# mx-mark/VideoTransformer-pytorch

Measured on NVIDIA H100. Metric: clips/sec (BxTx3x224x224) TimeSformer-B fwd+bwd, higher is better.
Workload: dtype bf16

## Files before the change

### videotransformer_pytorch_b200/csrc/vt_gemm.cu

```cuda
#include <stdlib.h>
#include <string.h>

#include "vt_common.cuh"
#include "vt_sm90.cuh"

namespace vt {

constexpr int BM = 128;
constexpr int BK = 64;
constexpr int GEMM_THREADS = 384;
constexpr int CHUNK_BYTES = 64 * BK * 2;

struct GemmDev {
  int M, N, K;
  int kblocks, splits;
  int num_m, num_n, tiles;
  int epi;
  const float* bias;
  const float* bias2;
  void* out;
  void* out2;
  const void* aux;
  long long ldo, ldo2, ldaux;
  const int* out_row;
  const int* aux_row;
  const float* row_scale;
  long long split_stride;
  int map_period, map_skip, map_tcount;
  long long map_stride_t, map_stride_p, map_stride_b, map_base;
  float* special_out;
  long long special_ld;
  const float* a_scale;
  const float* b_scale;
};

constexpr int EPI_BOX_BYTES = 64 * 64 * 2;

template <int BN, int SE>
struct GemmCfg {
  static constexpr int A_BYTES = BM * BK * 2;
  static constexpr int B_BYTES = BN * BK * 2;
  static constexpr int STAGE_BYTES = A_BYTES + B_BYTES;
  static constexpr int EPI_TILE_BYTES = BM * BN * 2;
  static constexpr int EPI_BYTES = SE * EPI_TILE_BYTES;
  static constexpr int SMEM_LIMIT = 232448, SMEM_EXTRA = 1024  + 256 ;
  static constexpr int STAGES_FIT = (SMEM_LIMIT - SMEM_EXTRA - EPI_BYTES) / STAGE_BYTES;
  static constexpr int STAGES = STAGES_FIT < 6 ? STAGES_FIT : 6;
  static constexpr int SMEM_BYTES = STAGES * STAGE_BYTES + EPI_BYTES + SMEM_EXTRA;
  static_assert(STAGES >= 2 && SMEM_BYTES <= SMEM_LIMIT, "shared memory budget");
};

template <int BN, int TA, int TB>
__device__ __forceinline__ void wgmma_tile(float (&acc)[BN / 2], uint64_t da, uint64_t db, uint32_t scale_d) {
  if constexpr (BN == 256) wgmma_m64n256k16<TA, TB>(acc, da, db, scale_d);
  else if constexpr (BN == 192) wgmma_m64n192k16<TA, TB>(acc, da, db, scale_d);
  else wgmma_m64n128k16<TA, TB>(acc, da, db, scale_d);
}

struct EpiRow {
  char* out;
  const char* aux;
  char* out2;
  float s;
};

__device__ __forceinline__ EpiRow epi_row(const GemmDev& p, int row, int split) {
  EpiRow r{nullptr, nullptr, nullptr, 1.0f};
  if (row >= p.M) return r;
  if (p.row_scale) r.s = p.row_scale[row];
  if (p.epi == VT_EPI_F32) {
    float* out = static_cast<float*>(p.out);
    const float* aux = static_cast<const float*>(p.aux);
    if (p.map_period > 0) {
      const int outer = row / p.map_period, inner = row - outer * p.map_period;
      if (inner < p.map_skip) {
        if (p.special_out) r.out = reinterpret_cast<char*>(p.special_out + (long long)outer * p.special_ld);
        return r;
      }
      const long long off = p.map_base + (long long)(outer % p.map_tcount) * p.map_stride_t +
                            (long long)(inner - p.map_skip) * p.map_stride_p + (long long)(outer / p.map_tcount) * p.map_stride_b;
      r.out = reinterpret_cast<char*>(out + off);
      r.aux = reinterpret_cast<const char*>(aux + off);
      return r;
    }
    const int orow = p.out_row ? p.out_row[row] : row;
    if (orow >= 0) r.out = reinterpret_cast<char*>(out + (long long)split * p.split_stride + (long long)orow * p.ldo);
    if (aux) {
      const int arow = p.aux_row ? p.aux_row[row] : row;
      if (arow >= 0) r.aux = reinterpret_cast<const char*>(aux + (long long)arow * p.ldaux);
    }
    return r;
  }
  const int orow = p.out_row ? p.out_row[row] : row;
  if (orow < 0) return r;
  r.out = reinterpret_cast<char*>(static_cast<__nv_bfloat16*>(p.out) + (long long)orow * p.ldo);
  if (p.epi == VT_EPI_GELU) r.out2 = reinterpret_cast<char*>(static_cast<__nv_bfloat16*>(p.out2) + (long long)orow * p.ldo2);
  if (p.epi == VT_EPI_DGELU) r.aux = reinterpret_cast<const char*>(static_cast<const __nv_bfloat16*>(p.aux) + (long long)row * p.ldaux);
// ... 44 lines not shown
__device__ __forceinline__ void epi_stage(const GemmDev& p, const float (&acc)[BN / 2], uint8_t* stage, uint8_t* stage2,
                                          int row0, int n0, int warp, int lane) {
  const int r = warp * 16 + (lane >> 2);
  float s[2] = {1.0f, 1.0f};
  if ((EPI == VT_EPI_BF16 || EPI == VT_EPI_GELU_H) && p.row_scale) {
#pragma unroll
    for (int h = 0; h < 2; ++h)
      if (row0 + r + 8 * h < p.M) s[h] = p.row_scale[row0 + r + 8 * h];
  }
  const uint32_t a1 = smem_u32(stage) + r * 128 + 4 * (lane & 3) + ((lane >> 2) << 4);
  const uint32_t a2 = smem_u32(stage2) + r * 128 + 4 * (lane & 3) + ((lane >> 2) << 4);
#pragma unroll
  for (int j = 0; j < BN / 8; ++j) {
    const int n = n0 + 8 * j + 2 * (lane & 3);
    if (n >= p.N) break;
#pragma unroll
    for (int h = 0; h < 2; ++h) {
      const uint32_t off = (j >> 3) * EPI_BOX_BYTES + h * 8 * 128;
      const uint32_t o = (a1 ^ ((j & 7) << 4)) + off, o2 = (a2 ^ ((j & 7) << 4)) + off;
      float v0 = acc[4 * j + 2 * h], v1 = acc[4 * j + 2 * h + 1];
      add_bias(p, n, v0, v1);
      if (EPI == VT_EPI_BF16) {
        st_shared_u32(o, pack_bf16x2(s[h] * v0, s[h] * v1));
      } else if (EPI == VT_EPI_GELU_H) {
        st_shared_u32(o, gelu_pair(pack_bf16x2(s[h] * v0, s[h] * v1)));
      } else if (EPI == VT_EPI_GELU) {
        const uint32_t z = pack_bf16x2(v0, v1);
        st_shared_u32(o, z);
        st_shared_u32(o2, gelu_pair(z));
      } else {
        st_shared_u32(o, dgelu_pair(ld_shared_u32(o2), v0, v1));
      }
    }
  }
}

struct Tile {
  int m0, n0, split, kb0, kb1;
};

template <int BN>
__device__ __forceinline__ Tile tile_at(const GemmDev& p, int t) {
  Tile c;
  const int nt = t % p.num_n, rest = t / p.num_n;
  const int mt = rest % p.num_m;
  c.split = rest / p.num_m;
  c.m0 = mt * BM;
  c.n0 = nt * BN;
  c.kb0 = (int)(((long long)p.kblocks * c.split) / p.splits);
  c.kb1 = (int)(((long long)p.kblocks * (c.split + 1)) / p.splits);
  return c;
}

template <int BN, int TA, int TB, int SE, int F8>
__device__ __forceinline__ void gemm_wgmma_body(const CUtensorMap& tmA, const CUtensorMap& tmB, const CUtensorMap& tmC,
                                                const CUtensorMap& tmD, const GemmDev& p) {
  using Cfg = GemmCfg<BN, SE>;
  static_assert(!F8 || (BN == 128 && !TA && !TB && SE < 2), "e4m3 forms: BN = 128, K-major operands, one output");
  constexpr int STAGES = Cfg::STAGES;
  constexpr int KB_ELEMS = F8 ? 128 : BK;
  constexpr int HALF_BYTES = Cfg::EPI_TILE_BYTES / 2;
  extern __shared__ uint8_t smem_raw[];
  uint8_t* smem = reinterpret_cast<uint8_t*>((reinterpret_cast<uintptr_t>(smem_raw) + 1023) & ~uintptr_t(1023));
  uint8_t* epi_smem = smem + STAGES * Cfg::STAGE_BYTES;
  uint64_t* full_bar = reinterpret_cast<uint64_t*>(epi_smem + Cfg::EPI_BYTES);
  uint64_t* empty_bar = full_bar + STAGES;
  uint64_t* zfull_bar = empty_bar + STAGES;
  uint64_t* zempty_bar = zfull_bar + 1;
  const bool load_z = SE == 2 && p.epi == VT_EPI_DGELU;

  const int wg = threadIdx.x >> 7;
  if (threadIdx.x == 0) {
    tma_prefetch_desc(&tmA);
    tma_prefetch_desc(&tmB);
    if (SE > 0) tma_prefetch_desc(&tmC);
    if (SE == 2) tma_prefetch_desc(&tmD);
    for (int i = 0; i < STAGES; ++i) {
      mbar_init(&full_bar[i], 1);
      mbar_init(&empty_bar[i], 8);
    }
    mbar_init(zfull_bar, 1);
    mbar_init(zempty_bar, 2);
    fence_barrier_init();
  }
  __syncthreads();

  if (wg == 0) {
    setmaxnreg_dec<40>();
    if (threadIdx.x == 0) {
      uint32_t it = 0;
      uint32_t tj = 0;
      for (int t = blockIdx.x; t < p.tiles; t += gridDim.x, ++tj) {
        const Tile c = tile_at<BN>(p, t);
        for (int kb = c.kb0; kb < c.kb1; ++kb, ++it) {
          const int stage = (int)(it % STAGES);
          mbar_wait(&empty_bar[stage], ((it / STAGES) & 1) ^ 1);
          uint8_t* sA = smem + stage * Cfg::STAGE_BYTES;
          uint8_t* sB = sA + Cfg::A_BYTES;
          mbar_arrive_expect_tx(&full_bar[stage], Cfg::STAGE_BYTES);
          if (!TA) {
            tma_load_2d(sA, &tmA, &full_bar[stage], kb * KB_ELEMS, c.m0);
          } else {
#pragma unroll
            for (int ch = 0; ch < BM / 64; ++ch) tma_load_2d(sA + ch * CHUNK_BYTES, &tmA, &full_bar[stage], c.m0 + ch * 64, kb * BK);
          }
          if (!TB) {
            tma_load_2d(sB, &tmB, &full_bar[stage], kb * KB_ELEMS, c.n0);
          } else {
#pragma unroll
            for (int ch = 0; ch < BN / 64; ++ch) tma_load_2d(sB + ch * CHUNK_BYTES, &tmB, &full_bar[stage], c.n0 + ch * 64, kb * BK);
          }
        }
        if (load_z) {
          mbar_wait(zempty_bar, (tj & 1) ^ 1);
          mbar_arrive_expect_tx(zfull_bar, Cfg::EPI_TILE_BYTES);
          uint8_t* zt = epi_smem + Cfg::EPI_TILE_BYTES;
#pragma unroll
          for (int h = 0; h < 2; ++h)
#pragma unroll
            for (int b = 0; b < BN / 64; ++b)
              tma_load_2d(zt + h * HALF_BYTES + b * EPI_BOX_BYTES, &tmD, zfull_bar, c.n0 + 64 * b, c.m0 + 64 * h);
        }
      }
    }
    return;
  }

  setmaxnreg_inc<232>();
  const int cw = wg - 1;
  const int warp = (threadIdx.x >> 5) & 3, lane = threadIdx.x & 31;
  const bool leader = (threadIdx.x & 127) == 0;
  uint8_t* stage = epi_smem + cw * HALF_BYTES;
  uint8_t* stage2 = stage + Cfg::EPI_TILE_BYTES;
  uint32_t it = 0, tj = 0;
  float part[F8 ? BN / 2 : 1];
#pragma unroll
  for (int i = 0; i < (F8 ? BN / 2 : 1); ++i) part[i] = 0.f;
  for (int t = blockIdx.x; t < p.tiles; t += gridDim.x, ++tj) {
    const Tile c = tile_at<BN>(p, t);
    float acc[BN / 2];
#pragma unroll
    for (int i = 0; i < BN / 2; ++i) acc[i] = 0.f;
    if constexpr (F8) {
      for (int kb = c.kb0; kb < c.kb1; ++kb, ++it) {
        const int stage = (int)(it % STAGES);
        mbar_wait(&full_bar[stage], (it / STAGES) & 1);
        const uint32_t a_addr = smem_u32(smem + stage * Cfg::STAGE_BYTES) + cw * 64 * 128;
        const uint32_t b_addr = smem_u32(smem + stage * Cfg::STAGE_BYTES + Cfg::A_BYTES);
        wgmma_fence();
#pragma unroll
        for (int k = 0; k < 4; ++k)
          wgmma_m64n128k32_e4m3(part, sdesc_kmajor(a_addr + k * 32), sdesc_kmajor(b_addr + k * 32), k > 0 ? 1u : 0u);
        wgmma_commit();
        wgmma_wait<0>();
        if (lane == 0) mbar_arrive(&empty_bar[stage]);
#pragma unroll
        for (int i = 0; i < BN / 2; ++i) acc[i] += part[i];
      }
      const int rr = c.m0 + cw * 64 + warp * 16 + (lane >> 2);
      const float sa0 = rr < p.M ? p.a_scale[rr] : 0.f, sa1 = rr + 8 < p.M ? p.a_scale[rr + 8] : 0.f;
#pragma unroll
      for (int j = 0; j < BN / 8; ++j) {
        const int n = c.n0 + 8 * j + 2 * (lane & 3);
        if (n >= p.N) break;
        const float2 sb = __ldg(reinterpret_cast<const float2*>(p.b_scale + n));
        acc[4 * j] *= sa0 * sb.x;
        acc[4 * j + 1] *= sa0 * sb.y;
        acc[4 * j + 2] *= sa1 * sb.x;
        acc[4 * j + 3] *= sa1 * sb.y;
      }
    } else {
    int prev = -1;
    for (int kb = c.kb0; kb < c.kb1; ++kb, ++it) {
      const int stage = (int)(it % STAGES);
      mbar_wait(&full_bar[stage], (it / STAGES) & 1);
      const uint32_t a_addr = smem_u32(smem + stage * Cfg::STAGE_BYTES) + cw * (TA ? CHUNK_BYTES : 64 * 128);
      const uint32_t b_addr = smem_u32(smem + stage * Cfg::STAGE_BYTES + Cfg::A_BYTES);
      wgmma_fence();
#pragma unroll
      for (int k = 0; k < BK / 16; ++k) {
        const uint64_t da = TA ? sdesc_mnmajor(a_addr + k * 2048, CHUNK_BYTES) : sdesc_kmajor(a_addr + k * 32);
        const uint64_t db = TB ? sdesc_mnmajor(b_addr + k * 2048, CHUNK_BYTES) : sdesc_kmajor(b_addr + k * 32);
        wgmma_tile<BN, TA, TB>(acc, da, db, (kb > c.kb0 || k > 0) ? 1u : 0u);
      }
      wgmma_commit();
      wgmma_wait<1>();
      if (prev >= 0 && lane == 0) mbar_arrive(&empty_bar[prev]);
      prev = stage;
    }
    wgmma_wait<0>();
    if (lane == 0) mbar_arrive(&empty_bar[prev]);
    }

    if constexpr (SE > 0) {
      const int row0 = c.m0 + cw * 64;
      if (load_z) mbar_wait(zfull_bar, tj & 1);
      if (leader) tma_store_wait_read_all();
      named_bar_sync(1 + cw, 128);
      if (SE == 1 && p.epi == VT_EPI_GELU_H) epi_stage<BN, VT_EPI_GELU_H>(p, acc, stage, stage2, row0, c.n0, warp, lane);
      else if (SE == 1) epi_stage<BN, VT_EPI_BF16>(p, acc, stage, stage2, row0, c.n0, warp, lane);
      else if (p.epi == VT_EPI_GELU) epi_stage<BN, VT_EPI_GELU>(p, acc, stage, stage2, row0, c.n0, warp, lane);
      else epi_stage<BN, VT_EPI_DGELU>(p, acc, stage, stage2, row0, c.n0, warp, lane);
      fence_proxy_async_smem();
      named_bar_sync(1 + cw, 128);
      if (leader) {
        if (load_z) mbar_arrive(zempty_bar);
        if (row0 < p.M) {
#pragma unroll
          for (int b = 0; b < BN / 64; ++b) {
            if (c.n0 + 64 * b >= p.N) break;
            tma_store_2d(&tmC, stage + b * EPI_BOX_BYTES, c.n0 + 64 * b, row0);
            if (SE == 2 && p.epi == VT_EPI_GELU) tma_store_2d(&tmD, stage2 + b * EPI_BOX_BYTES, c.n0 + 64 * b, row0);
          }
        }
        tma_store_commit();
      }
    } else {
      const int r0 = c.m0 + cw * 64 + warp * 16 + (lane >> 2);
      const EpiRow e0 = epi_row(p, r0, c.split), e1 = epi_row(p, r0 + 8, c.split);
#pragma unroll
      for (int j = 0; j < BN / 8; ++j) {
        const int n = c.n0 + 8 * j + 2 * (lane & 3);
        if (n >= p.N) break;
        epi_pair(p, e0, n, acc[4 * j], acc[4 * j + 1]);
        epi_pair(p, e1, n, acc[4 * j + 2], acc[4 * j + 3]);
      }
    }
  }
  if (SE > 0 && leader) tma_store_wait_read_all();
}

template <int BN, int TA, int TB, int SE>
__global__ void __launch_bounds__(GEMM_THREADS, 1)
gemm_wgmma_kernel(const __grid_constant__ CUtensorMap tmA, const __grid_constant__ CUtensorMap tmB,
                  const __grid_constant__ CUtensorMap tmC, const __grid_constant__ CUtensorMap tmD, const GemmDev p) {
  gemm_wgmma_body<BN, TA, TB, SE, 0>(tmA, tmB, tmC, tmD, p);
}

template <int SE>
__global__ void __launch_bounds__(GEMM_THREADS, 1)
gemm_e4m3_kernel(const __grid_constant__ CUtensorMap tmA, const __grid_constant__ CUtensorMap tmB,
                 const __grid_constant__ CUtensorMap tmC, const __grid_constant__ CUtensorMap tmD, const GemmDev p) {
  gemm_wgmma_body<128, 0, 0, SE, 1>(tmA, tmB, tmC, tmD, p);
}

typedef CUresult (*EncodeTiledFn)(CUtensorMap*, CUtensorMapDataType, cuuint32_t, void*, const cuuint64_t*,
                                  const cuuint64_t*, const cuuint32_t*, const cuuint32_t*, CUtensorMapInterleave,
                                  CUtensorMapSwizzle, CUtensorMapL2promotion, CUtensorMapFloatOOBfill);

static EncodeTiledFn get_encode_fn() {
  static EncodeTiledFn fn = nullptr;
  if (!fn) {
    void* ptr = nullptr;
    cudaDriverEntryPointQueryResult qres;
    cudaError_t e = cudaGetDriverEntryPoint("cuTensorMapEncodeTiled", &ptr, cudaEnableDefault, &qres);
    if (e != cudaSuccess || qres != cudaDriverEntryPointSuccess || !ptr) return nullptr;
    fn = reinterpret_cast<EncodeTiledFn>(ptr);
  }
  return fn;
}

static int make_tmap_2d(CUtensorMap* map, int esize, const void* base, long long rows, long long cols, long long ld,
                        int box_rows) {
  EncodeTiledFn fn = get_encode_fn();
  VT_REQUIRE(fn != nullptr, "cuTensorMapEncodeTiled entry point unavailable");
  VT_REQUIRE((reinterpret_cast<uintptr_t>(base) & 15) == 0, "TMA base pointer must be 16-byte aligned");
  VT_REQUIRE((ld * esize) % 16 == 0, "TMA leading dimension must be a multiple of %d elements (got %lld)", 16 / esize, ld);
  cuuint64_t gdim[2] = {(cuuint64_t)cols, (cuuint64_t)rows};
  cuuint64_t gstr[1] = {(cuuint64_t)(ld * esize)};
  cuuint32_t box[2] = {(cuuint32_t)(128 / esize), (cuuint32_t)box_rows};
  cuuint32_t estr[2] = {1u, 1u};
  CUresult r = fn(map, esize == 2 ? CU_TENSOR_MAP_DATA_TYPE_BFLOAT16 : CU_TENSOR_MAP_DATA_TYPE_UINT8, 2, const_cast<void*>(base),
                  gdim, gstr, box, estr,
                  CU_TENSOR_MAP_INTERLEAVE_NONE, CU_TENSOR_MAP_SWIZZLE_128B, CU_TENSOR_MAP_L2_PROMOTION_L2_256B,
                  CU_TENSOR_MAP_FLOAT_OOB_FILL_NONE);
  VT_REQUIRE(r == CUDA_SUCCESS, "cuTensorMapEncodeTiled failed (%d) rows=%lld cols=%lld ld=%lld box_rows=%d", (int)r,
             rows, cols, ld, box_rows);
  return 0;
}

int make_tmap_bf16_2d(CUtensorMap* map, const void* base, long long rows, long long cols, long long ld, int box_rows) {
  return make_tmap_2d(map, 2, base, rows, cols, ld, box_rows);
}

__global__ void reduce_rows_kernel(const float* __restrict__ in, float* __restrict__ out, long long stride, int S,
                                   long long n4, int accumulate, float scale) {
  for (long long i = blockIdx.x * (long long)blockDim.x + threadIdx.x; i < n4; i += (long long)gridDim.x * blockDim.x) {
    float4 acc = make_float4(0.f, 0.f, 0.f, 0.f);
    for (int s = 0; s < S; ++s) {
// ... 15 lines not shown
reduce_rows_tall_kernel(const float* __restrict__ in, float* __restrict__ out, long long stride, int S, long long n4,
                        int accumulate, float scale) {
  const int cq = threadIdx.x % RT_QUADS, rl = threadIdx.x / RT_QUADS;
  const long long i = blockIdx.x * (long long)RT_QUADS + cq;
  float4 acc = make_float4(0.f, 0.f, 0.f, 0.f);
  if (i < n4) {
    for (int s = rl; s < S; s += RT_LANES) {
      const float4 v = *reinterpret_cast<const float4*>(in + (long long)s * stride + i * 4);
      acc.x += v.x; acc.y += v.y; acc.z += v.z; acc.w += v.w;
    }
  }
  __shared__ float4 sh[RT_LANES][RT_QUADS];
  sh[rl][cq] = acc;
  __syncthreads();
  if (rl < 16) {
    float4 a = sh[rl][cq];
#pragma unroll
    for (int r = rl + 16; r < RT_LANES; r += 16) { a.x += sh[r][cq].x; a.y += sh[r][cq].y; a.z += sh[r][cq].z; a.w += sh[r][cq].w; }
    sh[rl][cq] = a;
  }
  __syncthreads();
  if (rl == 0 && i < n4) {
    float4 a = sh[0][cq];
#pragma unroll
    for (int r = 1; r < 16; ++r) { a.x += sh[r][cq].x; a.y += sh[r][cq].y; a.z += sh[r][cq].z; a.w += sh[r][cq].w; }
    a.x *= scale; a.y *= scale; a.z *= scale; a.w *= scale;
    float4* o = reinterpret_cast<float4*>(out + i * 4);
    if (accumulate) { const float4 p = *o; a.x += p.x; a.y += p.y; a.z += p.z; a.w += p.w; }
    *o = a;
  }
}

int launch_reduce_rows(const float* in, float* out, long long stride, int S, long long n, int accumulate, float scale,
                       cudaStream_t st) {
  VT_REQUIRE(n % 4 == 0 && stride % 4 == 0, "vt_reduce_rows: n and stride must be multiples of 4");
  const long long n4 = n / 4;
  if (S >= 32 && n4 <= 16 * 4096) {
    reduce_rows_tall_kernel<<<(int)((n4 + RT_QUADS - 1) / RT_QUADS), RT_QUADS * RT_LANES, 0, st>>>(in, out, stride, S, n4, accumulate, scale);
    return check_launch("reduce_rows_tall_kernel");
  }
  int blocks = (int)((n4 + 255) / 256);
  const int cap = sm_count() * 8;
  if (blocks > cap) blocks = cap;
  if (blocks < 1) blocks = 1;
  reduce_rows_kernel<<<blocks, 256, 0, st>>>(in, out, stride, S, n4, accumulate, scale);
  return check_launch("reduce_rows_kernel");
}

template <int BN, int TA, int TB, int SE, int F8 = 0>
static int launch_gemm_t(const CUtensorMap (&tm)[4], const GemmDev& d, cudaStream_t st) {
  using Cfg = GemmCfg<BN, SE>;
  void (*kernel)(const CUtensorMap, const CUtensorMap, const CUtensorMap, const CUtensorMap, const GemmDev);
  if constexpr (F8) kernel = gemm_e4m3_kernel<SE>;
  else kernel = gemm_wgmma_kernel<BN, TA, TB, SE>;
  static bool attr_set = false;
  if (!attr_set) {
    cudaError_t e = cudaFuncSetAttribute(kernel, cudaFuncAttributeMaxDynamicSharedMemorySize, Cfg::SMEM_BYTES);
    VT_REQUIRE(e == cudaSuccess, "cudaFuncSetAttribute(smem=%d) failed: %s", Cfg::SMEM_BYTES, cudaGetErrorString(e));
    attr_set = true;
  }
  const int grid = d.tiles < persistent_sm_count() ? d.tiles : persistent_sm_count();
  kernel<<<grid, GEMM_THREADS, Cfg::SMEM_BYTES, st>>>(tm[0], tm[1], tm[2], tm[3], d);
  return check_launch(F8 ? "gemm_e4m3_kernel" : "gemm_wgmma_kernel");
}

template <int BN, int SE>
static int launch_layout(const vt_gemm_params* q, const CUtensorMap (&tm)[4], const GemmDev& d, cudaStream_t st) {
  if (!q->a_mn_major && !q->b_mn_major) return launch_gemm_t<BN, 0, 0, SE>(tm, d, st);
  if (!q->a_mn_major) return launch_gemm_t<BN, 0, 1, SE>(tm, d, st);
  if (!q->b_mn_major) return launch_gemm_t<BN, 1, 0, SE>(tm, d, st);
  return launch_gemm_t<BN, 1, 1, SE>(tm, d, st);
}

#ifndef VT_DEFAULT_STAGED_EPI
#define VT_DEFAULT_STAGED_EPI true
#endif
static int staged_kind(const vt_gemm_params* q) {
  if (q->epilogue == VT_EPI_F32 || q->out_row) return 0;
  if (!feature_on("VT_GEMM_STAGED_EPI", VT_DEFAULT_STAGED_EPI)) return 0;
  if (q->epilogue == VT_EPI_BF16 || q->epilogue == VT_EPI_GELU_H) return 1;
  if (q->epilogue == VT_EPI_GELU && ((reinterpret_cast<uintptr_t>(q->out2) & 15) || (q->ldo2 * 2) % 16)) return 0;
  return 2;
}

template <int BN, int F8 = 0>
static int launch_gemm(const vt_gemm_params* q, GemmDev& d, cudaStream_t st) {
  CUtensorMap tm[4];
  memset(tm, 0, sizeof(tm));
  CUtensorMap &tmA = tm[0], &tmB = tm[1];
  int rc;
  if (F8) {
    rc = make_tmap_2d(&tmA, 1, q->a, q->M, q->K, q->lda, BM);
    if (!rc) rc = make_tmap_2d(&tmB, 1, q->b, q->N, q->K, q->ldb, BN);
  } else if (!q->a_mn_major) rc = make_tmap_bf16_2d(&tmA, q->a, q->M, q->K, q->lda, BM);
  else rc = make_tmap_bf16_2d(&tmA, q->a, q->K, q->M, q->lda, BK);
  if (rc) return rc;
  if (!F8) {
    if (!q->b_mn_major) rc = make_tmap_bf16_2d(&tmB, q->b, q->N, q->K, q->ldb, BN);
    else rc = make_tmap_bf16_2d(&tmB, q->b, q->K, q->N, q->ldb, BK);
    if (rc) return rc;
  }
  d.num_m = (q->M + BM - 1) / BM;
  d.num_n = (q->N + BN - 1) / BN;
  const long long tiles = (long long)d.num_m * d.num_n * d.splits;
  VT_REQUIRE(tiles < (1LL << 31), "vt_gemm: M=%d N=%d gives too many tiles", q->M, q->N);
  d.tiles = (int)tiles;
  const long long tile_out = (long long)q->M * q->N;
  void* final_out = d.out;
  d.split_stride = 0;
  if (d.splits > 1) {
    d.out = q->workspace;
    d.ldo = q->N;
    d.split_stride = tile_out;
  }
  const int se = d.splits > 1 ? 0 : staged_kind(q);
  if (se > 0) {
    rc = make_tmap_bf16_2d(&tm[2], q->out, q->M, q->N, q->ldo, 64);
    if (!rc && q->epilogue == VT_EPI_GELU) rc = make_tmap_bf16_2d(&tm[3], q->out2, q->M, q->N, q->ldo2, 64);
    if (!rc && q->epilogue == VT_EPI_DGELU) rc = make_tmap_bf16_2d(&tm[3], q->aux, q->M, q->N, q->ldaux, 64);
    if (rc) return rc;
  }
  if constexpr (F8) {
    rc = se == 1 ? launch_gemm_t<BN, 0, 0, 1, 1>(tm, d, st) : launch_gemm_t<BN, 0, 0, 0, 1>(tm, d, st);
  } else {
    if (se == 1) rc = launch_layout<BN, 1>(q, tm, d, st);
    else if (se == 2) rc = launch_layout<BN, 2>(q, tm, d, st);
    else rc = launch_layout<BN, 0>(q, tm, d, st);
  }
  if (rc) return rc;
  if (d.splits > 1) {
    VT_REQUIRE(q->ldo == q->N, "vt_gemm: split-K requires ldo == N");
    return launch_reduce_rows(static_cast<const float*>(q->workspace), static_cast<float*>(final_out), tile_out, d.splits, tile_out,
                              0, 1.0f, st);
  }
  return 0;
}

int launch_gemm_rows(const vt_gemm_params* q, int m0, void* stream);

}

#ifndef VT_DEFAULT_ROWS_SPLIT
#define VT_DEFAULT_ROWS_SPLIT false
#endif
static int rows_split_point(const vt_gemm_params* q) {
  const int r = q->M % vt::BM;
  if (r == 0 || r > 16 || q->M < 8 * vt::BM) return 0;
  if (q->N > 1024 || q->K < 2048) return 0;
  if (!vt::feature_on("VT_ROWS_SPLIT", VT_DEFAULT_ROWS_SPLIT)) return 0;
  if (q->a_mn_major || (q->epilogue != VT_EPI_BF16 && q->epilogue != VT_EPI_F32)) return 0;
  if (q->out_row || q->aux_row || q->map_period > 0 || q->debug || q->force_splits || q->force_bn || q->force_cluster || q->force_tail) return 0;
  if (q->epilogue == VT_EPI_F32 && q->workspace && !q->aux && !q->bias && !q->row_scale) return 0;
  if (q->K % 8 != 0 || q->lda % 8 != 0 || q->ldb % 8 != 0) return 0;
  if ((reinterpret_cast<uintptr_t>(q->a) & 15) || (reinterpret_cast<uintptr_t>(q->b) & 15)) return 0;
  return q->M - r;
}

static int gemm_dispatch(const vt_gemm_params* q, const float* a_scale, const float* b_scale, void* stream);

extern "C" int vt_gemm(const vt_gemm_params* q, void* stream) {
  using namespace vt;
  VT_REQUIRE(q != nullptr, "vt_gemm: null params");
  const int m0 = (q->a && q->b && q->out && q->M > 0 && q->N > 0 && q->K > 0) ? rows_split_point(q) : 0;
  if (m0 > 0) {
    vt_gemm_params head = *q;
    head.M = m0;
    const int rc = gemm_dispatch(&head, nullptr, nullptr, stream);
    if (rc) return rc;
    return launch_gemm_rows(q, m0, stream);
  }
  return gemm_dispatch(q, nullptr, nullptr, stream);
}

extern "C" int vt_gemm_e4m3(const vt_gemm_e4m3_params* p, void* stream) {
  using namespace vt;
  VT_REQUIRE(p != nullptr, "vt_gemm_e4m3: null params");
  const vt_gemm_params* q = &p->g;
  VT_REQUIRE(p->a_scale && p->b_scale && (reinterpret_cast<uintptr_t>(p->b_scale) & 15) == 0,
             "vt_gemm_e4m3: a_scale and b_scale are required (b_scale 16-byte aligned)");
  VT_REQUIRE(!q->a_mn_major && !q->b_mn_major, "vt_gemm_e4m3: both operands must be K-major");
// ... 15 lines not shown
  const bool f8 = a_scale != nullptr;
  VT_REQUIRE(q->M > 0 && q->N > 0 && q->K > 0, "vt_gemm: bad shape M=%d N=%d K=%d", q->M, q->N, q->K);
  VT_REQUIRE(q->N % 8 == 0, "vt_gemm: N must be a multiple of 8 (got %d)", q->N);
  VT_REQUIRE(q->a && q->b && q->out, "vt_gemm: null operand");
  VT_REQUIRE(q->epilogue >= VT_EPI_BF16 && q->epilogue <= VT_EPI_GELU_H, "vt_gemm: bad epilogue %d", q->epilogue);
  if (q->epilogue == VT_EPI_GELU) VT_REQUIRE(q->out2 != nullptr, "vt_gemm: VT_EPI_GELU needs out2");
  if (q->epilogue == VT_EPI_DGELU) VT_REQUIRE(q->aux != nullptr, "vt_gemm: VT_EPI_DGELU needs aux (z)");
  const int esz = (q->epilogue == VT_EPI_F32) ? 4 : 2;
  VT_REQUIRE((q->ldo * esz) % 16 == 0 && (reinterpret_cast<uintptr_t>(q->out) & 15) == 0,
             "vt_gemm: out must be 16B aligned with 16B-multiple row pitch");
  if (q->aux) VT_REQUIRE((reinterpret_cast<uintptr_t>(q->aux) & 15) == 0 && (q->ldaux * esz) % 16 == 0, "vt_gemm: aux misaligned");
  if (q->bias) VT_REQUIRE((reinterpret_cast<uintptr_t>(q->bias) & 15) == 0, "vt_gemm: bias misaligned");
  if (q->bias2) VT_REQUIRE(q->epilogue == VT_EPI_F32 && q->aux && (reinterpret_cast<uintptr_t>(q->bias2) & 15) == 0,
                           "vt_gemm: bias2 needs the fp32 epilogue with an addend, 16-byte aligned");
  VT_REQUIRE(q->force_bn == 0 || q->force_bn == 128 || q->force_bn == 192 || q->force_bn == 256,
             "vt_gemm: force_bn must be 128, 192 or 256");

  GemmDev d;
  d.M = q->M; d.N = q->N; d.K = q->K;
  d.epi = q->epilogue;
  d.bias = q->bias;
  d.bias2 = q->bias2;
  d.out = q->out; d.out2 = q->out2; d.aux = q->aux;
  d.ldo = q->ldo; d.ldo2 = q->ldo2; d.ldaux = q->ldaux;
  d.out_row = q->out_row; d.aux_row = q->aux_row; d.row_scale = q->row_scale;
  d.kblocks = f8 ? (q->K + 127) / 128 : (q->K + BK - 1) / BK;
  d.a_scale = a_scale; d.b_scale = b_scale;
  d.map_period = 0; d.map_skip = 0; d.map_tcount = 1;
  d.map_stride_t = d.map_stride_p = d.map_stride_b = d.map_base = 0;
  d.special_out = nullptr; d.special_ld = 0;
  if (q->map_period > 0) {
    VT_REQUIRE(q->epilogue == VT_EPI_F32 && q->aux, "vt_gemm: the affine row map applies to the fp32 residual epilogue only");
    VT_REQUIRE(q->M % q->map_period == 0 && q->map_tcount >= 1 && q->map_skip >= 0 && q->map_skip < q->map_period,
               "vt_gemm: bad affine row map (period %d, skip %d, tcount %d, M %d)", q->map_period, q->map_skip, q->map_tcount, q->M);
    VT_REQUIRE(q->map_base % 2 == 0 && q->map_stride_t % 2 == 0 && q->map_stride_p % 2 == 0 && q->map_stride_b % 2 == 0 &&
                   (q->map_special_base < 0 || (q->map_special_base % 2 == 0 && q->map_special_stride % 2 == 0)),
               "vt_gemm: affine row map offsets and strides must be even (8-byte aligned fp32 pairs)");
    d.map_period = q->map_period; d.map_skip = q->map_skip; d.map_tcount = q->map_tcount;
    d.map_stride_t = q->map_stride_t; d.map_stride_p = q->map_stride_p; d.map_stride_b = q->map_stride_b; d.map_base = q->map_base;
    d.special_out = q->map_special_base >= 0 ? static_cast<float*>(q->out) + q->map_special_base : nullptr;
    d.special_ld = q->map_special_stride;
  }

  if (f8) {
    d.splits = 1;
    return launch_gemm<128, 1>(q, d, static_cast<cudaStream_t>(stream));
  }
  const bool short_k = d.kblocks <= 16;
  const bool one_staged = staged_kind(q) == 1;
  const int sms = persistent_sm_count();
  const int num_m = (q->M + BM - 1) / BM;
  const bool can_split = q->epilogue == VT_EPI_F32 && q->workspace && !q->out_row && !q->aux && !q->row_scale && !q->bias &&
                         q->map_period == 0;
  const int cand[3] = {256, 192, 128};
  const double penalty[3] = {1.0, 1.04, 1.10};
  double best = 1e30;
  int bn = 128, splits = 1;
  for (int i = 0; i < 3; ++i) {
    if (q->force_bn && cand[i] != q->force_bn) continue;
    if (!q->force_bn && !can_split && short_k && cand[i] != 128 && !(one_staged && cand[i] == 192)) continue;
    const int num_n = (q->N + cand[i] - 1) / cand[i];
    const int smax = can_split ? 16 : 1;
    for (int sp = 1; sp <= smax; ++sp) {
      if (sp > 1 && (d.kblocks / sp < 4 || (long long)sp * q->M * q->N * 4 > q->workspace_bytes)) break;
      const long long tiles = (long long)num_m * num_n * sp;
      const double per_cta = (double)((tiles + sms - 1) / sms);
      const double cost = per_cta * ((double)d.kblocks / sp + 8.0) * cand[i] * penalty[i];
      if (cost < best - 1e-9) { best = cost; bn = cand[i]; splits = sp; }
    }
  }
  if (can_split && q->force_splits > 0) {
    splits = q->force_splits;
    const long long max_by_ws = q->workspace_bytes / ((long long)q->M * q->N * 4);
    if (splits > max_by_ws) splits = (int)max_by_ws;
    if (splits > d.kblocks) splits = d.kblocks;
    if (splits < 1) splits = 1;
  }
  d.splits = splits;
  cudaStream_t st = static_cast<cudaStream_t>(stream);
  if (bn == 256) return launch_gemm<256>(q, d, st);
  if (bn == 192) return launch_gemm<192>(q, d, st);
  return launch_gemm<128>(q, d, st);
}

extern "C" int vt_reduce_rows(const vt_reduce_params* p, void* stream) {
  using namespace vt;
  VT_REQUIRE(p && p->in && p->out && p->S >= 1, "vt_reduce_rows: bad params");
  return launch_reduce_rows(p->in, p->out, p->stride, p->S, p->n, p->accumulate, p->scale,
                            static_cast<cudaStream_t>(stream));
}
```

### videotransformer_pytorch_b200/csrc/vt_sm90.cuh

```cuda
#pragma once
#include <cuda.h>
#include <cuda_bf16.h>
#include <cuda_runtime.h>
#include <stdint.h>

namespace vt {

__device__ __forceinline__ uint32_t smem_u32(const void* p) {
  return static_cast<uint32_t>(__cvta_generic_to_shared(p));
}

__device__ __forceinline__ void st_shared_u32(uint32_t addr, uint32_t v) {
  asm volatile("st.shared.b32 [%0], %1;" ::"r"(addr), "r"(v) : "memory");
}
__device__ __forceinline__ uint32_t ld_shared_u32(uint32_t addr) {
  uint32_t v;
  asm volatile("ld.shared.b32 %0, [%1];" : "=r"(v) : "r"(addr) : "memory");
  return v;
}

__device__ __forceinline__ void mbar_init(uint64_t* bar, uint32_t count) {
  asm volatile("mbarrier.init.shared::cta.b64 [%0], %1;" ::"r"(smem_u32(bar)), "r"(count));
}
__device__ __forceinline__ void fence_barrier_init() {
  asm volatile("fence.mbarrier_init.release.cluster;" ::: "memory");
}
__device__ __forceinline__ void mbar_arrive_expect_tx(uint64_t* bar, uint32_t bytes) {
  asm volatile("mbarrier.arrive.expect_tx.shared::cta.b64 _, [%0], %1;" ::"r"(smem_u32(bar)), "r"(bytes)
               : "memory");
}
__device__ __forceinline__ void mbar_arrive(uint64_t* bar) {
  asm volatile("mbarrier.arrive.shared::cta.b64 _, [%0];" ::"r"(smem_u32(bar)) : "memory");
}
__device__ __forceinline__ bool mbar_try_wait(uint64_t* bar, uint32_t parity) {
  uint32_t ok;
  asm volatile(
      "{\n\t.reg .pred P;\n\t"
      "mbarrier.try_wait.parity.shared::cta.b64 P, [%1], %2;\n\t"
      "selp.b32 %0, 1, 0, P;\n\t}\n"
      : "=r"(ok)
      : "r"(smem_u32(bar)), "r"(parity)
      : "memory");
  return ok != 0;
}
__device__ __forceinline__ void mbar_wait(uint64_t* bar, uint32_t parity) {
  uint32_t spins = 0;
  while (!mbar_try_wait(bar, parity)) {
    if (++spins > (1u << 28)) __trap();
  }
}

__device__ __forceinline__ void tma_prefetch_desc(const CUtensorMap* m) {
  asm volatile("prefetch.tensormap [%0];" ::"l"(reinterpret_cast<uint64_t>(m)) : "memory");
}
__device__ __forceinline__ void tma_load_2d(void* smem_dst, const CUtensorMap* map, uint64_t* bar, int c0,
                                            int c1) {
  asm volatile(
      "cp.async.bulk.tensor.2d.shared::cluster.global.mbarrier::complete_tx::bytes [%0], [%1, {%3, %4}], [%2];"
      ::"r"(smem_u32(smem_dst)),
      "l"(reinterpret_cast<uint64_t>(map)), "r"(smem_u32(bar)), "r"(c0), "r"(c1)
      : "memory");
}
__device__ __forceinline__ void tma_store_2d(const CUtensorMap* map, const void* smem_src, int c0, int c1) {
  asm volatile("cp.async.bulk.tensor.2d.global.shared::cta.bulk_group [%0, {%2, %3}], [%1];"
               ::"l"(reinterpret_cast<uint64_t>(map)), "r"(smem_u32(smem_src)), "r"(c0), "r"(c1)
               : "memory");
}
__device__ __forceinline__ void tma_store_commit() { asm volatile("cp.async.bulk.commit_group;" ::: "memory"); }
__device__ __forceinline__ void tma_store_wait_read_all() {
  asm volatile("cp.async.bulk.wait_group.read 0;" ::: "memory");
}
__device__ __forceinline__ void fence_proxy_async_smem() { asm volatile("fence.proxy.async.shared::cta;" ::: "memory"); }
__device__ __forceinline__ void named_bar_sync(int id, int count) {
  asm volatile("bar.sync %0, %1;" ::"r"(id), "r"(count) : "memory");
}

__device__ __forceinline__ void wgmma_fence() { asm volatile("wgmma.fence.sync.aligned;" ::: "memory"); }
__device__ __forceinline__ void wgmma_commit() { asm volatile("wgmma.commit_group.sync.aligned;" ::: "memory"); }
template <int N>
__device__ __forceinline__ void wgmma_wait() {
  asm volatile("wgmma.wait_group.sync.aligned %0;" ::"n"(N) : "memory");
}
template <int R>
__device__ __forceinline__ void setmaxnreg_inc() { asm volatile("setmaxnreg.inc.sync.aligned.u32 %0;" ::"n"(R)); }
template <int R>
__device__ __forceinline__ void setmaxnreg_dec() { asm volatile("setmaxnreg.dec.sync.aligned.u32 %0;" ::"n"(R)); }

__device__ __forceinline__ uint64_t make_sdesc_sw128(uint32_t smem_addr, uint32_t lbo_bytes, uint32_t sbo_bytes) {
  uint64_t d = 0;
  d |= static_cast<uint64_t>((smem_addr & 0x3FFFF) >> 4);
  d |= static_cast<uint64_t>((lbo_bytes >> 4) & 0x3FFF) << 16;
  d |= static_cast<uint64_t>((sbo_bytes >> 4) & 0x3FFF) << 32;
  d |= static_cast<uint64_t>(1) << 62;
  return d;
}
__device__ __forceinline__ uint64_t sdesc_kmajor(uint32_t addr) { return make_sdesc_sw128(addr, 16, 1024); }
__device__ __forceinline__ uint64_t sdesc_mnmajor(uint32_t addr, uint32_t chunk_bytes) {
  return make_sdesc_sw128(addr, chunk_bytes, 1024);
}

template <int TA, int TB>
__device__ __forceinline__ void wgmma_m64n128k16(float (&d)[64], uint64_t da, uint64_t db, uint32_t scale_d) {
  asm volatile(
      "{\n\t.reg .pred p;\n\t"
      "setp.ne.b32 p, %66, 0;\n\t"
      "wgmma.mma_async.sync.aligned.m64n128k16.f32.bf16.bf16 "
      "{%0,%1,%2,%3,%4,%5,%6,%7,%8,%9,%10,%11,%12,%13,%14,%15,%16,%17,%18,%19,%20,%21,%22,%23,%24,%25,%26,%27,%28,%29,%30,%31,%32,%33,%34,%35,%36,%37,%38,%39,%40,%41,%42,%43,%44,%45,%46,%47,%48,%49,%50,%51,%52,%53,%54,%55,%56,%57,%58,%59,%60,%61,%62,%63}, "
      "%64, %65, p, 1, 1, %67, %68;\n\t}\n"
      : "+f"(d[0]), "+f"(d[1]), "+f"(d[2]), "+f"(d[3]), "+f"(d[4]), "+f"(d[5]), "+f"(d[6]), "+f"(d[7]), "+f"(d[8]), "+f"(d[9]), "+f"(d[10]), "+f"(d[11]), "+f"(d[12]), "+f"(d[13]), "+f"(d[14]), "+f"(d[15]), "+f"(d[16]), "+f"(d[17]), "+f"(d[18]), "+f"(d[19]), "+f"(d[20]), "+f"(d[21]), "+f"(d[22]), "+f"(d[23]), "+f"(d[24]), "+f"(d[25]), "+f"(d[26]), "+f"(d[27]), "+f"(d[28]), "+f"(d[29]), "+f"(d[30]), "+f"(d[31]), "+f"(d[32]), "+f"(d[33]), "+f"(d[34]), "+f"(d[35]), "+f"(d[36]), "+f"(d[37]), "+f"(d[38]), "+f"(d[39]), "+f"(d[40]), "+f"(d[41]), "+f"(d[42]), "+f"(d[43]), "+f"(d[44]), "+f"(d[45]), "+f"(d[46]), "+f"(d[47]), "+f"(d[48]), "+f"(d[49]), "+f"(d[50]), "+f"(d[51]), "+f"(d[52]), "+f"(d[53]), "+f"(d[54]), "+f"(d[55]), "+f"(d[56]), "+f"(d[57]), "+f"(d[58]), "+f"(d[59]), "+f"(d[60]), "+f"(d[61]), "+f"(d[62]), "+f"(d[63])
      : "l"(da), "l"(db), "r"(scale_d), "n"(TA), "n"(TB));
}

template <int TA, int TB>
__device__ __forceinline__ void wgmma_m64n192k16(float (&d)[96], uint64_t da, uint64_t db, uint32_t scale_d) {
  asm volatile(
      "{\n\t.reg .pred p;\n\t"
      "setp.ne.b32 p, %98, 0;\n\t"
      "wgmma.mma_async.sync.aligned.m64n192k16.f32.bf16.bf16 "
// ... 31 lines not shown
```

Baseline: 240.5.

## Stage fp32 GEMM epilogue through shared memory with bulk row copies

Adds an fp32 staged-epilogue mode. Two idle producer-warpgroup warps bulk-load the residual (aux) rows into a padded shared-memory tile. The consumer warpgroups then add bias, scale and the residual into that tile, and the same warps write each row back with 1D bulk async stores. This replaces scattered per-thread fp32 global loads and stores in the residual/fp32-output epilogues. The price is extra shared memory for the staging tile, which leaves fewer pipeline stages, a ban on BN=256 for this path, and new barrier handshakes that could serialize tiles.

Result: faster. 262.5 (median of 6 runs) (+9.1%).

```diff
diff --git a/videotransformer_pytorch_b200/csrc/vt_gemm.cu b/videotransformer_pytorch_b200/csrc/vt_gemm.cu
--- a/videotransformer_pytorch_b200/csrc/vt_gemm.cu
+++ b/videotransformer_pytorch_b200/csrc/vt_gemm.cu
@@ -35,6 +35,7 @@
 };
 
 constexpr int EPI_BOX_BYTES = 64 * 64 * 2;
+constexpr int SE_F32 = 3;
 
 template <int BN, int SE>
 struct GemmCfg {
@@ -42,7 +43,8 @@
   static constexpr int B_BYTES = BN * BK * 2;
   static constexpr int STAGE_BYTES = A_BYTES + B_BYTES;
   static constexpr int EPI_TILE_BYTES = BM * BN * 2;
-  static constexpr int EPI_BYTES = SE * EPI_TILE_BYTES;
+  static constexpr int F32_PITCH = BN + 8;
+  static constexpr int EPI_BYTES = SE == SE_F32 ? BM * F32_PITCH * 4 : SE * EPI_TILE_BYTES;
   static constexpr int SMEM_LIMIT = 232448, SMEM_EXTRA = 1024  + 256 ;
   static constexpr int STAGES_FIT = (SMEM_LIMIT - SMEM_EXTRA - EPI_BYTES) / STAGE_BYTES;
   static constexpr int STAGES = STAGES_FIT < 6 ? STAGES_FIT : 6;
@@ -193,11 +195,80 @@
   return c;
 }
 
+template <int BN>
+__device__ __forceinline__ void epi_f32_io(const GemmDev& p, float* stage, uint64_t* full, uint64_t* ready, int half, int lane) {
+  constexpr int PITCH = GemmCfg<BN, SE_F32>::F32_PITCH;
+  uint32_t tj = 0;
+  for (int t = blockIdx.x; t < p.tiles; t += gridDim.x, ++tj) {
+    const Tile c = tile_at<BN>(p, t);
+    const int cols = p.N - c.n0 < BN ? p.N - c.n0 : BN;
+    const uint32_t bytes = (uint32_t)cols * 4;
+    const int row0 = c.m0 + half * 64 + lane;
+    const EpiRow e0 = epi_row(p, row0, c.split), e1 = epi_row(p, row0 + 32, c.split);
+    float* s0 = stage + lane * PITCH;
+    float* s1 = s0 + 32 * PITCH;
+    tma_store_wait_read_all();
+    uint32_t tx = 0;
+    if (p.aux) {
+      if (e0.out && e0.aux) tx += bytes;
+      if (e1.out && e1.aux) tx += bytes;
+      for (int h = 0; h < 2; ++h) {
+        const EpiRow& e = h ? e1 : e0;
+        if (e.out && !e.aux)
+          for (int i = 0; i < cols; i += 4) st_shared_zero16(smem_u32((h ? s1 : s0) + i));
+      }
+    }
+    mbar_arrive_expect_tx(full, tx);
+    if (tx) {
+      if (e0.out && e0.aux) bulk_load_1d(s0, reinterpret_cast<const float*>(e0.aux) + c.n0, bytes, full);
+      if (e1.out && e1.aux) bulk_load_1d(s1, reinterpret_cast<const float*>(e1.aux) + c.n0, bytes, full);
+    }
+    mbar_wait(ready, tj & 1);
+    if (e0.out) bulk_store_1d(reinterpret_cast<float*>(e0.out) + c.n0, s0, bytes);
+    if (e1.out) bulk_store_1d(reinterpret_cast<float*>(e1.out) + c.n0, s1, bytes);
+    tma_store_commit();
+  }
+  tma_store_wait_read_all();
+}
+
+template <int BN>
+__device__ __forceinline__ void epi_f32_stage(const GemmDev& p, const float (&acc)[BN / 2], const float* stage, int row0, int n0,
+                                              int warp, int lane) {
+  constexpr int PITCH = GemmCfg<BN, SE_F32>::F32_PITCH;
+  const int r = warp * 16 + (lane >> 2);
+  float s[2] = {1.0f, 1.0f};
+  if (p.row_scale) {
+#pragma unroll
+    for (int h = 0; h < 2; ++h)
+      if (row0 + r + 8 * h < p.M) s[h] = p.row_scale[row0 + r + 8 * h];
+  }
+  const uint32_t a0 = smem_u32(stage + r * PITCH + 2 * (lane & 3));
+#pragma unroll
+  for (int j = 0; j < BN / 8; ++j) {
+    const int n = n0 + 8 * j + 2 * (lane & 3);
+    if (n >= p.N) break;
+#pragma unroll
+    for (int h = 0; h < 2; ++h) {
+      const uint32_t o = a0 + (h * 8 * PITCH + 8 * j) * 4;
+      float v0 = acc[4 * j + 2 * h], v1 = acc[4 * j + 2 * h + 1];
+      add_bias(p, n, v0, v1);
+      float2 a = make_float2(0.f, 0.f);
+      if (p.aux) a = ld_shared_f32x2(o);
+      if (p.bias2) {
+        const float2 b2 = __ldg(reinterpret_cast<const float2*>(p.bias2 + n));
+        a.x += b2.x; a.y += b2.y;
+      }
+      st_shared_f32x2(o, fmaf(s[h], v0, a.x), fmaf(s[h], v1, a.y));
+    }
+  }
+}
+
 template <int BN, int TA, int TB, int SE, int F8>
 __device__ __forceinline__ void gemm_wgmma_body(const CUtensorMap& tmA, const CUtensorMap& tmB, const CUtensorMap& tmC,
                                                 const CUtensorMap& tmD, const GemmDev& p) {
   using Cfg = GemmCfg<BN, SE>;
-  static_assert(!F8 || (BN == 128 && !TA && !TB && SE < 2), "e4m3 forms: BN = 128, K-major operands, one output");
+  static_assert(!F8 || (BN == 128 && !TA && !TB && SE != 2), "e4m3 forms: BN = 128, K-major operands, one output");
+  static_assert(SE != SE_F32 || BN != 256, "the fp32 staging tile leaves too few ring stages at BN = 256");
   constexpr int STAGES = Cfg::STAGES;
   constexpr int KB_ELEMS = F8 ? 128 : BK;
   constexpr int HALF_BYTES = Cfg::EPI_TILE_BYTES / 2;
@@ -208,13 +279,15 @@
   uint64_t* empty_bar = full_bar + STAGES;
   uint64_t* zfull_bar = empty_bar + STAGES;
   uint64_t* zempty_bar = zfull_bar + 1;
+  uint64_t* rows_full_bar = zempty_bar + 1;
+  uint64_t* rows_ready_bar = rows_full_bar + 2;
   const bool load_z = SE == 2 && p.epi == VT_EPI_DGELU;
 
   const int wg = threadIdx.x >> 7;
   if (threadIdx.x == 0) {
     tma_prefetch_desc(&tmA);
     tma_prefetch_desc(&tmB);
-    if (SE > 0) tma_prefetch_desc(&tmC);
+    if (SE == 1 || SE == 2) tma_prefetch_desc(&tmC);
     if (SE == 2) tma_prefetch_desc(&tmD);
     for (int i = 0; i < STAGES; ++i) {
       mbar_init(&full_bar[i], 1);
@@ -222,12 +295,23 @@
     }
     mbar_init(zfull_bar, 1);
     mbar_init(zempty_bar, 2);
+    for (int h = 0; h < 2; ++h) {
+      mbar_init(&rows_full_bar[h], 32);
+      mbar_init(&rows_ready_bar[h], 128);
+    }
     fence_barrier_init();
   }
   __syncthreads();
 
   if (wg == 0) {
     setmaxnreg_dec<40>();
+    const int pw = threadIdx.x >> 5;
+    if constexpr (SE == SE_F32) {
+      if (pw == 1 || pw == 2) {
+        float* rows = reinterpret_cast<float*>(epi_smem) + (pw - 1) * 64 * Cfg::F32_PITCH;
+        epi_f32_io<BN>(p, rows, &rows_full_bar[pw - 1], &rows_ready_bar[pw - 1], pw - 1, threadIdx.x & 31);
+      }
+    }
     if (threadIdx.x == 0) {
       uint32_t it = 0;
       uint32_t tj = 0;
@@ -333,7 +417,13 @@
     if (lane == 0) mbar_arrive(&empty_bar[prev]);
     }
 
-    if constexpr (SE > 0) {
+    if constexpr (SE == SE_F32) {
+      const float* rows = reinterpret_cast<const float*>(epi_smem) + cw * 64 * Cfg::F32_PITCH;
+      mbar_wait(&rows_full_bar[cw], tj & 1);
+      epi_f32_stage<BN>(p, acc, rows, c.m0 + cw * 64, c.n0, warp, lane);
+      fence_proxy_async_smem();
+      mbar_arrive(&rows_ready_bar[cw]);
+    } else if constexpr (SE > 0) {
       const int row0 = c.m0 + cw * 64;
       if (load_z) mbar_wait(zfull_bar, tj & 1);
       if (leader) tma_store_wait_read_all();
@@ -368,7 +458,7 @@
       }
     }
   }
-  if (SE > 0 && leader) tma_store_wait_read_all();
+  if ((SE == 1 || SE == 2) && leader) tma_store_wait_read_all();
 }
 
 template <int BN, int TA, int TB, int SE>
@@ -376,6 +466,13 @@
 gemm_wgmma_kernel(const __grid_constant__ CUtensorMap tmA, const __grid_constant__ CUtensorMap tmB,
                   const __grid_constant__ CUtensorMap tmC, const __grid_constant__ CUtensorMap tmD, const GemmDev p) {
   gemm_wgmma_body<BN, TA, TB, SE, 0>(tmA, tmB, tmC, tmD, p);
+}
+
+template <int BN, int TA, int TB>
+__global__ void __launch_bounds__(GEMM_THREADS, 1)
+gemm_f32_kernel(const __grid_constant__ CUtensorMap tmA, const __grid_constant__ CUtensorMap tmB,
+                const __grid_constant__ CUtensorMap tmC, const __grid_constant__ CUtensorMap tmD, const GemmDev p) {
+  gemm_wgmma_body<BN, TA, TB, SE_F32, 0>(tmA, tmB, tmC, tmD, p);
 }
 
 template <int SE>
@@ -497,6 +594,7 @@
   using Cfg = GemmCfg<BN, SE>;
   void (*kernel)(const CUtensorMap, const CUtensorMap, const CUtensorMap, const CUtensorMap, const GemmDev);
   if constexpr (F8) kernel = gemm_e4m3_kernel<SE>;
+  else if constexpr (SE == SE_F32) kernel = gemm_f32_kernel<BN, TA, TB>;
   else kernel = gemm_wgmma_kernel<BN, TA, TB, SE>;
   static bool attr_set = false;
   if (!attr_set) {
@@ -506,7 +604,7 @@
   }
   const int grid = d.tiles < persistent_sm_count() ? d.tiles : persistent_sm_count();
   kernel<<<grid, GEMM_THREADS, Cfg::SMEM_BYTES, st>>>(tm[0], tm[1], tm[2], tm[3], d);
-  return check_launch(F8 ? "gemm_e4m3_kernel" : "gemm_wgmma_kernel");
+  return check_launch(F8 ? "gemm_e4m3_kernel" : SE == SE_F32 ? "gemm_f32_kernel" : "gemm_wgmma_kernel");
 }
 
 template <int BN, int SE>
@@ -521,8 +619,15 @@
 #define VT_DEFAULT_STAGED_EPI true
 #endif
 static int staged_kind(const vt_gemm_params* q) {
-  if (q->epilogue == VT_EPI_F32 || q->out_row) return 0;
   if (!feature_on("VT_GEMM_STAGED_EPI", VT_DEFAULT_STAGED_EPI)) return 0;
+  if (q->epilogue == VT_EPI_F32) {
+    if (q->map_period > 0 &&
+        (q->map_base % 4 || q->map_stride_t % 4 || q->map_stride_p % 4 || q->map_stride_b % 4 ||
+         (q->map_special_base >= 0 && (q->map_special_base % 4 || q->map_special_stride % 4))))
+      return 0;
+    return SE_F32;
+  }
+  if (q->out_row) return 0;
   if (q->epilogue == VT_EPI_BF16 || q->epilogue == VT_EPI_GELU_H) return 1;
   if (q->epilogue == VT_EPI_GELU && ((reinterpret_cast<uintptr_t>(q->out2) & 15) || (q->ldo2 * 2) % 16)) return 0;
   return 2;
@@ -558,19 +663,27 @@
     d.ldo = q->N;
     d.split_stride = tile_out;
   }
-  const int se = d.splits > 1 ? 0 : staged_kind(q);
-  if (se > 0) {
+  int se = staged_kind(q);
+  if (se == SE_F32 && (BN == 256 || (d.splits > 1 && (BN != 128 || (reinterpret_cast<uintptr_t>(q->workspace) & 15))))) se = 0;
+  if (se == 1 || se == 2) {
     rc = make_tmap_bf16_2d(&tm[2], q->out, q->M, q->N, q->ldo, 64);
     if (!rc && q->epilogue == VT_EPI_GELU) rc = make_tmap_bf16_2d(&tm[3], q->out2, q->M, q->N, q->ldo2, 64);
     if (!rc && q->epilogue == VT_EPI_DGELU) rc = make_tmap_bf16_2d(&tm[3], q->aux, q->M, q->N, q->ldaux, 64);
     if (rc) return rc;
   }
   if constexpr (F8) {
-    rc = se == 1 ? launch_gemm_t<BN, 0, 0, 1, 1>(tm, d, st) : launch_gemm_t<BN, 0, 0, 0, 1>(tm, d, st);
+    if (se == 1) rc = launch_gemm_t<BN, 0, 0, 1, 1>(tm, d, st);
+    else if (se == SE_F32) rc = launch_gemm_t<BN, 0, 0, SE_F32, 1>(tm, d, st);
+    else rc = launch_gemm_t<BN, 0, 0, 0, 1>(tm, d, st);
   } else {
     if (se == 1) rc = launch_layout<BN, 1>(q, tm, d, st);
     else if (se == 2) rc = launch_layout<BN, 2>(q, tm, d, st);
-    else rc = launch_layout<BN, 0>(q, tm, d, st);
+    else if constexpr (BN != 256) {
+      if (se == SE_F32) rc = launch_layout<BN, SE_F32>(q, tm, d, st);
+      else rc = launch_layout<BN, 0>(q, tm, d, st);
+    } else {
+      rc = launch_layout<BN, 0>(q, tm, d, st);
+    }
   }
   if (rc) return rc;
   if (d.splits > 1) {
@@ -692,13 +805,15 @@
   const int num_m = (q->M + BM - 1) / BM;
   const bool can_split = q->epilogue == VT_EPI_F32 && q->workspace && !q->out_row && !q->aux && !q->row_scale && !q->bias &&
                          q->map_period == 0;
+  const bool f32_staged = staged_kind(q) == SE_F32 && !can_split;
   const int cand[3] = {256, 192, 128};
   const double penalty[3] = {1.0, 1.04, 1.10};
   double best = 1e30;
   int bn = 128, splits = 1;
   for (int i = 0; i < 3; ++i) {
     if (q->force_bn && cand[i] != q->force_bn) continue;
-    if (!q->force_bn && !can_split && short_k && cand[i] != 128 && !(one_staged && cand[i] == 192)) continue;
+    if (!q->force_bn && !can_split && short_k && cand[i] != 128 && !((one_staged || f32_staged) && cand[i] == 192)) continue;
+    if (!q->force_bn && f32_staged && cand[i] == 256) continue;
     const int num_n = (q->N + cand[i] - 1) / cand[i];
     const int smax = can_split ? 16 : 1;
     for (int sp = 1; sp <= smax; ++sp) {
diff --git a/videotransformer_pytorch_b200/csrc/vt_sm90.cuh b/videotransformer_pytorch_b200/csrc/vt_sm90.cuh
--- a/videotransformer_pytorch_b200/csrc/vt_sm90.cuh
+++ b/videotransformer_pytorch_b200/csrc/vt_sm90.cuh
@@ -17,6 +17,17 @@
   uint32_t v;
   asm volatile("ld.shared.b32 %0, [%1];" : "=r"(v) : "r"(addr) : "memory");
   return v;
+}
+__device__ __forceinline__ void st_shared_f32x2(uint32_t addr, float x, float y) {
+  asm volatile("st.shared.v2.f32 [%0], {%1, %2};" ::"r"(addr), "f"(x), "f"(y) : "memory");
+}
+__device__ __forceinline__ float2 ld_shared_f32x2(uint32_t addr) {
+  float2 v;
+  asm volatile("ld.shared.v2.f32 {%0, %1}, [%2];" : "=f"(v.x), "=f"(v.y) : "r"(addr) : "memory");
+  return v;
+}
+__device__ __forceinline__ void st_shared_zero16(uint32_t addr) {
+  asm volatile("st.shared.v4.u32 [%0], {%1, %1, %1, %1};" ::"r"(addr), "r"(0u) : "memory");
 }
 
 __device__ __forceinline__ void mbar_init(uint64_t* bar, uint32_t count) {
@@ -64,6 +75,16 @@
 __device__ __forceinline__ void tma_store_2d(const CUtensorMap* map, const void* smem_src, int c0, int c1) {
   asm volatile("cp.async.bulk.tensor.2d.global.shared::cta.bulk_group [%0, {%2, %3}], [%1];"
                ::"l"(reinterpret_cast<uint64_t>(map)), "r"(smem_u32(smem_src)), "r"(c0), "r"(c1)
+               : "memory");
+}
+__device__ __forceinline__ void bulk_load_1d(void* smem_dst, const void* gsrc, uint32_t bytes, uint64_t* bar) {
+  asm volatile("cp.async.bulk.shared::cluster.global.mbarrier::complete_tx::bytes [%0], [%1], %2, [%3];"
+               ::"r"(smem_u32(smem_dst)), "l"(reinterpret_cast<uint64_t>(gsrc)), "r"(bytes), "r"(smem_u32(bar))
+               : "memory");
+}
+__device__ __forceinline__ void bulk_store_1d(void* gdst, const void* smem_src, uint32_t bytes) {
+  asm volatile("cp.async.bulk.global.shared::cta.bulk_group [%0], [%1], %2;"
+               ::"l"(reinterpret_cast<uint64_t>(gdst)), "r"(smem_u32(smem_src)), "r"(bytes)
                : "memory");
 }
 __device__ __forceinline__ void tma_store_commit() { asm volatile("cp.async.bulk.commit_group;" ::: "memory"); }
```
